# frgfm/Holocron

Measured on AMD Instinct MI355X. Metric: images/sec fwd+bwd+AdaBelief, RepVGG-A0 bs256/GPU 224^2, higher is better.
Workload: dtype bf16; 1 GPU; repvgg_a0 bf16 train step (fwd+bwd+AdaBelief), synthetic 224^2, bs=256 per MI355X (BASELINE.json configs[1]), random-init weights, 10 classes, CE label_smoothing 0.1; global_batch=256, parallelism=dp1, mode=weight gradients on a second stream; hipGraph replay of the full step, dump_outputs=/tmp/code/gt15__hip_graft__frgfm__Holocron/driver_out/dump_parent, deterministic=True

## Files before the change

holocron_amd/_lib.py:

```python
import ctypes as C
import os

import torch

_HERE = os.path.dirname(os.path.abspath(__file__))
LIB_PATH = os.environ.get("HC_LIB_PATH") or os.path.join(_HERE, "lib", "libholocron_hip.so")

HC_MAX_TAPS = 12
HC_MT_CHUNK = 8192
HC_STAT_REPLICAS = 128

c_void_p, c_int32, c_int64, c_float, c_double = C.c_void_p, C.c_int32, C.c_int64, C.c_float, C.c_double


class ConvClass(C.Structure):
    _fields_ = [("OHg", c_int32), ("OWg", c_int32), ("oy0", c_int32), ("ox0", c_int32), ("ostep", c_int32),
                ("istep", c_int32), ("ntaps", c_int32), ("tap", c_int32 * HC_MAX_TAPS)]


class ConvDesc(C.Structure):
    _fields_ = [("src0", c_void_p), ("src1", c_void_p), ("wpk", c_void_p), ("dst", c_void_p), ("resid", c_void_p),
                ("stats", c_void_p), ("bias", c_void_p), ("act", c_int32),
                ("N", c_int32), ("IH", c_int32), ("IW", c_int32), ("srcC", c_int32),
                ("OH", c_int32), ("OW", c_int32), ("Cout", c_int32), ("T", c_int32), ("nclass", c_int32),
# ... 162 lines not shown
    "hc_yolo1_loss_fwd": (c_int32, [c_void_p] * 3 + [c_int32] * 8 + [c_void_p] * 4 + [c_int32] + [c_void_p] * 4),
    "hc_yolo1_loss_bwd": (c_int32, [c_void_p] * 3 + [c_int32] * 8 + [c_void_p] * 4 + [c_int32] + [c_void_p] * 7),
    "hc_yolo1_decode": (c_int32, [c_void_p] * 3 + [c_int32] * 7 + [c_void_p] * 4),
    "hc_yolo_format_fwd": (c_int32, [c_void_p] * 2 + [c_int32] * 7 + [c_void_p] * 5),
    "hc_yolo_format_bwd": (c_int32, [c_void_p] * 3 + [c_int32] * 7 + [c_void_p] * 7),
    "hc_lamb_step": (c_int32, [c_void_p, c_int32, c_void_p, c_void_p, c_void_p, c_int32, c_void_p]),
    "hc_tadam_step": (c_int32, [c_void_p, c_int32, c_void_p, c_void_p, c_void_p, c_void_p, c_void_p, c_void_p, c_int32, c_void_p]),
    "hc_adan_step": (c_int32, [c_void_p, c_void_p, c_int32, c_void_p, c_void_p]),
    "hc_lookahead_sync": (c_int32, [c_void_p, c_int32, c_float, c_void_p]),
    "hc_multi_copy": (c_int32, [C.POINTER(MultiCopyDesc), c_void_p]),
    "hc_msbn_finalize": (c_int32, [C.POINTER(MsbnDesc), c_void_p]),
    "hc_msbn_bwd_finalize": (c_int32, [C.POINTER(MsbnDesc), c_void_p]),
    "hc_msbn_apply": (c_int32, [C.POINTER(MsbnIo), c_void_p, c_void_p, c_void_p, c_int32, c_void_p]),
    "hc_msbn_bwd_reduce": (c_int32, [C.POINTER(MsbnIo), c_void_p, c_int32, c_void_p, c_void_p, c_int32, c_void_p]),
    "hc_msbn_bwd_apply": (c_int32, [C.POINTER(MsbnIo), c_void_p, c_int32, c_void_p, c_void_p, c_int32, c_void_p]),
    "hc_dwrep_dgrad": (c_int32, [c_void_p, c_void_p, c_int32, c_void_p, c_void_p] + [c_int32] * 5 + [c_void_p]),
    "hc_conv_gather": (c_int32, [C.POINTER(ConvDesc), c_void_p]),
    "hc_conv_pointwise_supported": (c_int32, [C.POINTER(ConvDesc)]),
    "hc_conv_pointwise": (c_int32, [C.POINTER(ConvDesc), c_void_p]),
    "hc_conv_small": (c_int32, [C.POINTER(ConvSmallDesc), c_void_p]),
    "hc_conv_small_supported": (c_int32, [C.POINTER(ConvSmallDesc)]),
    "hc_conv_rows_fused_bwd_supported": (c_int32, [C.POINTER(ConvSmallDesc)]),
    "hc_conv_rows_fused_bwd": (c_int32, [C.POINTER(ConvSmallDesc), c_void_p, c_void_p, c_int32] + [c_void_p] * 8),
    "hc_conv_s2_supported": (c_int32, [C.POINTER(ConvS2Desc)]),
    "hc_conv_s2_fwd": (c_int32, [C.POINTER(ConvS2Desc), c_void_p]),
    "hc_conv_s2_dgrad_supported": (c_int32, [C.POINTER(ConvS2DgradDesc)]),
    "hc_conv_s2_dgrad": (c_int32, [C.POINTER(ConvS2DgradDesc), c_void_p]),
    "hc_conv_s2_stem_wgrad_ws_bytes": (c_int64, []),
    "hc_conv_s2_stem_wgrad": (c_int32, [c_void_p] * 6 + [c_int32] * 4 + [c_void_p]),
    "hc_conv_wgrad_ws_bytes": (c_int64, [C.POINTER(WgradDesc)]),
    "hc_conv_wgrad": (c_int32, [C.POINTER(WgradDesc), c_void_p]),
    "hc_conv_wgrad_group_supported": (c_int32, [C.POINTER(WgradGroupDesc)]),
    "hc_conv_wgrad_group_ws_bytes": (c_int64, [C.POINTER(WgradGroupDesc)]),
    "hc_conv_wgrad_group": (c_int32, [C.POINTER(WgradGroupDesc), c_void_p]),
    "hc_rep_wgrad_supported": (c_int32, [C.POINTER(RepWgradDesc)]),
    "hc_rep_wgrad_ws_bytes": (c_int64, [C.POINTER(RepWgradDesc)]),
    "hc_rep_wgrad_plan": (c_int32, [C.POINTER(RepWgradDesc), c_void_p]),
    "hc_rep_wgrad": (c_int32, [C.POINTER(RepWgradDesc), c_void_p]),
    "hc_pack_conv_weight": (c_int32, [c_void_p, c_void_p] + [c_int32] * 7 + [c_void_p]),
    "hc_pack_conv_weights_multi": (c_int32, [c_void_p, c_int32, c_int64, c_void_p]),
    "hc_nchw_to_nhwc_bf16": (c_int32, [c_void_p, c_void_p] + [c_int32] * 5 + [c_void_p]),
    "hc_nhwc_bf16_to_nchw": (c_int32, [c_void_p, c_void_p] + [c_int32] * 5 + [c_void_p]),
    "hc_im2col_small": (c_int32, [c_void_p, c_void_p] + [c_int32] * 11 + [c_void_p]),
    "hc_unpack_im2col_grad": (c_int32, [c_void_p, c_void_p] + [c_int32] * 6 + [c_void_p]),
    "hc_rep_bn_finalize": (c_int32, [C.POINTER(RepBnDesc), c_void_p]),
    "hc_rep_apply": (c_int32, [c_void_p] * 6 + [c_int64, c_int32, c_int32, c_void_p]),
# ... 152 lines not shown
```

holocron_amd/csrc/conv_rows48.hip:

```cpp
#include <type_traits>
#include "common.h"
#include "../../include/holocron_hip.h"

namespace crq {

constexpr int NT = 512, C = 48, CK = 2, PSC = C / 8 + 1, PS = PSC * 16, S3 = 9 * CK, S1 = CK, S = S3 + S1;
static_assert((PS / 8) % 4 == 2, "pixel pitch must be 2 x odd 8-byte units");

struct Args {
    hc_conv_small_desc d;
    int reps;
    int nunits;
    int delay;
};

template <int W>
struct Geo {
    static constexpr int RW = W > 64 ? 1 : 2;
    static constexpr int SEGW = (W + 15) / 16;
    static constexpr int NF = RW * SEGW;
    static constexpr int UR = 4 * RW;
    static constexpr int WW = W + 1;
    static constexpr int NSLOT = (UR + 2) * WW + 1;
    static constexpr int NDMA = (NSLOT * PS + 1023) / 1024;
    static constexpr int WIN = NDMA * 1024;
    static constexpr int SMEM = 2 * WIN + 64 + 1024;
    static_assert(SMEM <= 160 * 1024, "LDS budget");
};

__device__ __forceinline__ u32x4 uniform_rsrc(const void* p, unsigned bytes) {
    const unsigned long long v = reinterpret_cast<unsigned long long>(p);
    u32x4 r;
    r[0] = __builtin_amdgcn_readfirstlane((unsigned)v);
    r[1] = __builtin_amdgcn_readfirstlane((unsigned)(v >> 32) & 0xffffu);
    r[2] = __builtin_amdgcn_readfirstlane(bytes);
    r[3] = 0x00020000u;
    return r;
}
__device__ __forceinline__ bf16x8 frag2(const char* lo_p, const char* hi_p) {
    const u32x2 lo = *reinterpret_cast<const u32x2*>(lo_p), hi = *reinterpret_cast<const u32x2*>(hi_p);
    const u32x4 v = {lo[0], lo[1], hi[0], hi[1]};
    return __builtin_bit_cast(bf16x8, v);
}
__device__ __forceinline__ float row16_sum(float v) {
    v += __builtin_bit_cast(float, __builtin_amdgcn_update_dpp(0, __builtin_bit_cast(int, v), 0x128, 0xf, 0xf, false));
    v += __builtin_bit_cast(float, __builtin_amdgcn_update_dpp(0, __builtin_bit_cast(int, v), 0x124, 0xf, 0xf, false));
    v += __builtin_bit_cast(float, __builtin_amdgcn_update_dpp(0, __builtin_bit_cast(int, v), 0x122, 0xf, 0xf, false));
    v += __builtin_bit_cast(float, __builtin_amdgcn_update_dpp(0, __builtin_bit_cast(int, v), 0x121, 0xf, 0xf, false));
    return v;
}

template <int W, int MODE, int DBG>
__global__ __launch_bounds__(NT, 1) void conv_rows48_kernel(const Args a) {
    using G = Geo<W>;
    constexpr int WW = G::WW, NF = G::NF, UR = G::UR, RW = G::RW, SEGW = G::SEGW;
    extern __shared__ __attribute__((aligned(1024))) char smem[];
    const hc_conv_small_desc& d = a.d;
    const int tid = threadIdx.x, lane = tid & 63;
    const int wid = __builtin_amdgcn_readfirstlane(tid >> 6);
    const int team = wid >> 2, pw = wid & 3;
    const int H = d.H, UPI = H / UR;
    const unsigned lds0 = hc_lds_addr(smem);
    const int px = lane & 15, g = lane >> 4;
    const int region = team * G::WIN;
    int* cnt = reinterpret_cast<int*>(smem + 2 * G::WIN) + team * 8;
    int gen = 0;

    if (tid < 16) reinterpret_cast<int*>(smem + 2 * G::WIN)[tid] = 0;
    __syncthreads();

    auto team_sync = [&]() __attribute__((always_inline)) {
        asm volatile("s_waitcnt vmcnt(0) lgkmcnt(0)" ::: "memory");
        gen += 4;
        if (lane == 0) __hip_atomic_fetch_add(cnt, 1, __ATOMIC_RELAXED, __HIP_MEMORY_SCOPE_WORKGROUP);
        while (__hip_atomic_load(cnt, __ATOMIC_RELAXED, __HIP_MEMORY_SCOPE_WORKGROUP) < gen) __builtin_amdgcn_s_sleep(1);
        asm volatile("" ::: "memory");
    };

    const unsigned act_bytes = (unsigned)d.N * H * W * C * 2u;
    const u32x4 rsA = uniform_rsrc(d.srcA, act_bytes);
    const u32x4 rsB = uniform_rsrc(MODE == 1 ? d.srcB : d.srcA, act_bytes);
    const __amdgpu_buffer_rsrc_t rsw = make_rsrc(d.w3, (unsigned)(S * C * 64));

    const unsigned wl = (unsigned)((lane & 15) * 64 + g * 16);
    u32x4 af[3][3];
    auto load_a = [&](int buf, int s) __attribute__((always_inline)) {
        if (DBG & 4) return;
#pragma unroll
        for (int f = 0; f < 3; ++f) af[buf][f] = buf_load16(rsw, wl, (unsigned)(s * (C * 64) + f * 1024));
    };

    auto stage_window = [&](const u32x4 rs, int n, int row0, int j0, int j1) __attribute__((always_inline)) {
        if (DBG & 8) return;
        const unsigned img = (unsigned)n * (unsigned)(H * W * C * 2);
        for (int j = j0 + pw; j < j1; j += 4) {
            const int J = j * 64 + lane;
            const int slot = J / PSC, c = J - slot * PSC;
            const int r = slot / WW, x = slot - r * WW;
            const int ih = row0 - 1 + r;
            const bool ok = c < PSC - 1 && slot < G::NSLOT && x >= 1 && ih >= 0 && ih < H;
            const unsigned off = img + (unsigned)((ih * W + x - 1) * C * 2 + c * 16);
            hc_dma16(rs, lds0 + (unsigned)(region + j * 1024), ok ? off : HC_OOB);
        }
    };

    const int vb = region + ((pw * RW + 1) * WW + px + 1) * PS + g * 8;
    bf16x8 bfr[2][NF];
    auto load_b = [&](int buf, int bofs, int second) __attribute__((always_inline)) {
        if (DBG & 2) return;
        const char* sb = smem + vb + bofs;
#pragma unroll
        for (int i = 0; i < NF; ++i) {
            const int o = ((i / SEGW) * WW + 16 * (i % SEGW)) * PS;
            bfr[buf][i] = frag2(sb + o, sb + o + second);
        }
    };

    f32x4 acc[3][NF];
    auto zero_acc = [&]() __attribute__((always_inline)) {
#pragma unroll
        for (int f = 0; f < 3; ++f)
#pragma unroll
            for (int i = 0; i < NF; ++i) acc[f][i] = f32x4{0.f, 0.f, 0.f, 0.f};
    };
    auto mfma_step = [&](int ab, int bb) __attribute__((always_inline)) {
#pragma unroll
        for (int i = 0; i < NF; ++i)
#pragma unroll
            for (int f = 0; f < 3; ++f) {
                if (DBG & 1) acc[f][i][0] += __builtin_bit_cast(float, af[ab][f][0]) * (float)bfr[bb][i][0];
                else acc[f][i] = __builtin_amdgcn_mfma_f32_16x16x32_bf16(__builtin_bit_cast(bf16x8, af[ab][f]), bfr[bb][i], acc[f][i], 0, 0, 0);
            }
    };
    auto step = [&](int a3, int par, int s, int bnext, int second_next, bool prefetch) __attribute__((always_inline)) {
        if (s + 2 < S) load_a((a3 + 2) % 3, s + 2);
        if (prefetch) load_b(par ^ 1, bnext, second_next);
        __builtin_amdgcn_sched_barrier(0);
// ... 8 lines not shown
#pragma unroll
            for (int f = 0; f < 3; ++f)
#pragma unroll
                for (int i = 0; i < NF; ++i) t += acc[f][i][0];
            if (t == 123.456f) reinterpret_cast<float*>(outp)[tid] = t;
            return;
        }
        const size_t img = (size_t)n * H * W * C;
        __builtin_amdgcn_sched_barrier(0);
        float st[2][12];
#pragma unroll
        for (int k = 0; k < 2; ++k)
#pragma unroll
            for (int e = 0; e < 12; ++e) st[k][e] = 0.f;
#pragma unroll
        for (int i = 0; i < NF; ++i) {
            const int row = row0 + pw * RW + i / SEGW, col = 16 * (i % SEGW) + px;
            const bool ok = col < W;
            const size_t e0 = img + (size_t)(row * W + (ok ? col : 0)) * C + cbase;
            bf16_t* op = reinterpret_cast<bf16_t*>(outp) + e0;
            const bf16_t* rp = residp != nullptr ? reinterpret_cast<const bf16_t*>(residp) + e0 : nullptr;
            u32x4 r16 = {0u, 0u, 0u, 0u};
            u32x2 r8 = {0u, 0u};
            if (rp != nullptr && ok) {
                r16 = *reinterpret_cast<const u32x4*>(rp);
                r8 = *reinterpret_cast<const u32x2*>(rp + 32 - 4 * g);
            }
            u32x2 pk[3];
#pragma unroll
            for (int f = 0; f < 3; ++f) {
                f32x4 v = acc[f][i];
                if (stats != nullptr) {
#pragma unroll
                    for (int e = 0; e < 4; ++e) {
                        const float x = ok ? v[e] : 0.f;
                        st[0][f * 4 + e] += x;
                        st[1][f * 4 + e] += x * x;
                    }
                }
                const unsigned ra = f == 0 ? r16[0] : (f == 1 ? r16[2] : r8[0]), rb = f == 0 ? r16[1] : (f == 1 ? r16[3] : r8[1]);
                v[0] += bf16lo(ra); v[1] += bf16hi(ra); v[2] += bf16lo(rb); v[3] += bf16hi(rb);
                pk[f] = u32x2{pack_bf16x2(v[0], v[1]), pack_bf16x2(v[2], v[3])};
            }
            if (ok) {
                *reinterpret_cast<u32x4*>(op) = u32x4{pk[0][0], pk[0][1], pk[1][0], pk[1][1]};
                *reinterpret_cast<u32x2*>(op + 32 - 4 * g) = pk[2];
            }
        }
        if (stats != nullptr) {
            float* rep = stats + (size_t)((blockIdx.x * 8 + wid) % a.reps) * 2 * C + cbase;
#pragma unroll
            for (int k = 0; k < 2; ++k) {
                float mine = 0.f;
#pragma unroll
                for (int e = 0; e < 12; ++e) {
                    const float x = row16_sum(st[k][e]);
                    mine = px == e ? x : mine;
                }
                if (px < 12) atomicAdd(rep + k * C + (px < 8 ? px : 24 - 4 * g + px), mine);
            }
        }
    };

    if (team == 1)
        for (int i = 0; i < a.delay; ++i) __builtin_amdgcn_s_sleep(64);
    bool first = true;
    for (int u = 2 * blockIdx.x + team; u < a.nunits; u += 2 * gridDim.x) {
        const int n = u / UPI, row0 = (u - n * UPI) * UR;
        if (!first) team_sync();
        first = false;
        stage_window(rsA, n, row0, 0, G::NDMA);
        load_a(0, 0);
        load_a(1, 1);
        team_sync();
        zero_acc();
        load_b(0, (-WW - 1) * PS, 32);
#pragma nounroll
        for (int kh = 0; kh < 3; ++kh) {
            const int rofs = (kh - 1) * WW * PS;
#pragma unroll
            for (int t = 0; t < 6; ++t) {
                const int kw = t >> 1, kk = t & 1;
                int bnext, second;
                bool pf = true;
                if (kk == 0) { bnext = rofs + (kw - 1) * PS + 64; second = 0; }
                else if (t < 5) { bnext = rofs + kw * PS; second = 32; }
                else {
                    bnext = kh < 2 ? kh * WW * PS - PS : 0;
                    second = 32;
                    pf = kh < 2 || MODE == 0;
                }
                step(t % 3, kk, 6 * kh + t, bnext, second, pf);
            }
        }
        if (MODE == 0) {
            epilogue(d.out3, d.stats3, nullptr, n, row0);
            zero_acc();
        } else {
            team_sync();
            stage_window(rsB, n, row0, (WW * PS) / 1024, ((UR + 1) * WW * PS + PS + 1023) / 1024);
            team_sync();
            load_b(0, 0, 32);
        }
        step(0, 0, S3, 64, 0, true);
        step(1, 1, S3 + 1, 0, 0, false);
        if (MODE == 0) epilogue(d.out1, d.stats1, nullptr, n, row0);
        else epilogue(d.out3, nullptr, d.resid, n, row0);
    }
}

template <int W>
bool shape_ok(const hc_conv_small_desc& d) {
    return d.C == C && d.Cout == C && d.W == W && d.H >= Geo<W>::UR && d.H % Geo<W>::UR == 0 && d.N >= 1 &&
           (double)d.N * d.H * d.W * C * 2.0 < 2147483000.0;
}

template <int W, int MODE, int DBG>
void launch1(const Args& a, hipStream_t st) {
    auto kern = conv_rows48_kernel<W, MODE, DBG>;
    constexpr int smem = Geo<W>::SMEM;
    static bool attr_set = false;
    if (!attr_set) {
        (void)hipFuncSetAttribute(reinterpret_cast<const void*>(kern), hipFuncAttributeMaxDynamicSharedMemorySize, smem);
        attr_set = true;
    }
    int grid = (a.nunits + 1) / 2;
    if (grid > 256) grid = 256;
    hipLaunchKernelGGL(kern, dim3(grid), dim3(NT), smem, st, a);
}

template <int W>
void launch(Args& a, hipStream_t st) {
    static const int dbg = getenv("HC_CRQ_DBG") ? atoi(getenv("HC_CRQ_DBG")) : 0;
    constexpr int delay = 2;
    a.nunits = a.d.N * (a.d.H / Geo<W>::UR);
    a.delay = delay;
    const bool dg = (a.d.mode & 1) == 1;
#define CRQ_CASE(k) case k: if (dg) launch1<W, 1, k>(a, st); else launch1<W, 0, k>(a, st); break;
    switch (dbg) {
        CRQ_CASE(1) CRQ_CASE(2) CRQ_CASE(4) CRQ_CASE(7) CRQ_CASE(8) CRQ_CASE(16) CRQ_CASE(24) CRQ_CASE(31)
        default: if (dg) launch1<W, 1, 0>(a, st); else launch1<W, 0, 0>(a, st); break;
    }
#undef CRQ_CASE
}

}

bool hc_conv_rows48_supported(const hc_conv_small_desc& d) {
    static const int on = [] { const char* e = getenv("HC_CONV_ROWS48"); return e == nullptr ? 1 : atoi(e); }();
    if (on <= 0 || (d.mode & HC_CONV_SMALL_ROWS_IMAGE) == 0 || (d.mode & ~(HC_CONV_SMALL_ROWS_IMAGE | 1)) != 0) return false;
    if ((d.mode & 1) && on < 2) return false;
    return crq::shape_ok<112>(d) || crq::shape_ok<56>(d);
}
int hc_conv_rows48_launch(const hc_conv_small_desc& d, hipStream_t st) {
    if (!hc_conv_rows48_supported(d)) return HC_ERR_ARG;
    const bool dg = (d.mode & 1) == 1;
    if (d.srcA == nullptr || d.w3 == nullptr || d.out3 == nullptr) return HC_ERR_ARG;
    if (!dg && d.out1 == nullptr) return HC_ERR_ARG;
    if (dg && d.srcB == nullptr) return HC_ERR_ARG;
    if (!dg && (d.stats3 == nullptr) != (d.stats1 == nullptr)) return HC_ERR_ARG;
    crq::Args a;
    a.d = d;
    a.reps = hc_get_stat_replicas();
    if (d.W == 112) crq::launch<112>(a, st);
    else crq::launch<56>(a, st);
    return hc_launch_status();
}
```

holocron_amd/nn/repblock_op.py:

```python
import ctypes as C

import os

import torch

from .. import _lib
from .._lib import ConvS2Desc, ConvS2DgradDesc, PackItem, RepBnBwdDesc, RepBnDesc, StemBwdDesc, StemDesc, check, ptr, stream
from ..ops import conv as cv

STEM_KPAD = 32
FUSED_BWD = os.environ.get("HC_REP_FUSED_BWD", "1") != "0"


class ZeroPool:

    def __init__(self):
        self.buf = None
        self.used = 0
        self.high = 0
        self.depth = 0
        self.gen = 0
        self.retired = []
        self.graph_users = 0
        self.buf_captured = False

    def _retire(self):
        if self.buf is not None and self.buf_captured:
            self.retired.append(self.buf)
        self.buf, self.buf_captured = None, False

    def release_retired(self):
        self.graph_users = max(0, self.graph_users - 1)
        if self.graph_users == 0:
            self.retired = []
# ... 85 lines not shown
class RepState:

    def __init__(self, stride, identity):
        self.stride = stride
        self.identity = identity
        self.emit_stats = False
        self.fwd_cache = cv.PackCache()
        self.bwd_cache = cv.PackCache()
        self.desc = {}
        self.bn = None
        self.eps = 1e-5
        self.momentum = 0.1
        self.training = True
        self.last_out_stats = None
        self.packed = None
        self.packed_key = None
        self.pack_table = {}
        self.rows_image = (False, False)
        self.stack_fwd = False
        self.s2 = False
        self.s2_images = None
        self.s2_dgrad = False
        self.s2_dimg = None

    @staticmethod
    def weights_key(w3, w1):
        return (w3.data_ptr(), w3._version, w1.data_ptr(), w1._version, cv.weights_epoch())

    def pack_items(self, w3, w1):
        Cout, Cin = w3.shape[0], w3.shape[1]
        dev = w3.device
        stem = (Cin % 16) != 0
        if self.s2:
            return self._pack_items_s2(w3, w1, Cout, Cin, dev, stem)
        self.stack_fwd = (stem or (self.stride == 2 and Cin <= 48)) and Cout % 4 == 0
        if self.packed is None or self.packed[0].device != dev:
            if self.stack_fwd:
                self.packed = (torch.zeros((2 * Cout, 1, STEM_KPAD) if stem else (2 * Cout, 9, Cin), dtype=torch.bfloat16, device=dev),
                               None, None if stem else torch.empty((Cin, 10, Cout), dtype=torch.bfloat16, device=dev))
            elif any(self.rows_image):
                rf, rb = self.rows_image
                self.packed = (cv.rows_image(Cout, dev) if rf else torch.empty((Cout, 9, Cin), dtype=torch.bfloat16, device=dev),
                               None if rf else torch.empty((Cout, 1, Cin), dtype=torch.bfloat16, device=dev),
                               cv.rows_image(Cout, dev) if rb else torch.empty((Cin, 10, Cout), dtype=torch.bfloat16, device=dev))
            elif stem:
                self.packed = (torch.zeros((Cout, 1, STEM_KPAD), dtype=torch.bfloat16, device=dev),
                               torch.zeros((Cout, 1, STEM_KPAD), dtype=torch.bfloat16, device=dev), None)
            else:
                self.packed = (torch.empty((Cout, 9, Cin), dtype=torch.bfloat16, device=dev),
                               torch.empty((Cout, 1, Cin), dtype=torch.bfloat16, device=dev),
                               torch.empty((Cin, 10, Cout), dtype=torch.bfloat16, device=dev))
            self.packed_key = None
        wp3, wp1, wpd = self.packed
        if self.stack_fwd:
            if stem:
                return [(w3, wp3, Cout, Cin, 3, 3, 2, 0, STEM_KPAD), (w1, wp3[Cout:], Cout, Cin, 1, 1, 2, 4 * Cin, STEM_KPAD)]
            return [(w3, wp3, Cout, Cin, 3, 3, 0, 0, 9), (w1, wp3[Cout:], Cout, Cin, 1, 1, 0, 4, 9),
                    (w3, wpd, Cout, Cin, 3, 3, 1, 0, 10), (w1, wpd, Cout, Cin, 1, 1, 1, 9, 10)]
        if any(self.rows_image):
            rf, rb = self.rows_image
            fwd = ([(w3, wp3, Cout, Cin, 3, 3, 3, 0, 10), (w1, wp3, Cout, Cin, 1, 1, 3, 9, 10)] if rf else
                   [(w3, wp3, Cout, Cin, 3, 3, 0, 0, 9), (w1, wp1, Cout, Cin, 1, 1, 0, 0, 1)])
            bwd = ([(w3, wpd, Cout, Cin, 3, 3, 4, 0, 10), (w1, wpd, Cout, Cin, 1, 1, 4, 9, 10)] if rb else
                   [(w3, wpd, Cout, Cin, 3, 3, 1, 0, 10), (w1, wpd, Cout, Cin, 1, 1, 1, 9, 10)])
            return fwd + bwd
        if stem:
            return [(w3, wp3, Cout, Cin, 3, 3, 2, 0, STEM_KPAD), (w1, wp1, Cout, Cin, 1, 1, 2, 4 * Cin, STEM_KPAD)]
        return [(w3, wp3, Cout, Cin, 3, 3, 0, 0, 9), (w1, wp1, Cout, Cin, 1, 1, 0, 0, 1),
                (w3, wpd, Cout, Cin, 3, 3, 1, 0, 10), (w1, wpd, Cout, Cin, 1, 1, 1, 9, 10)]

    def _pack_items_s2(self, w3, w1, Cout, Cin, dev, stem):
        if stem:
            s3, s1, s1b, mode, tap1 = 2, 1, 0, 6, 4
        else:
            pt = Cin // 8
            s3, s1b, mode, tap1 = (9 * pt + 3) // 4, (9 * pt) // 4, 5, 9 * pt
            s1 = (10 * pt + 3) // 4 - s1b
        if self.s2_images is None or self.s2_images[0].device != dev:
            self.s2_images = (torch.zeros((Cout // 16, s3, 64, 8), dtype=torch.bfloat16, device=dev),
                              torch.zeros((Cout // 16, s1, 64, 8), dtype=torch.bfloat16, device=dev))
            self.packed_key = None
        gather_dgrad = not stem and not self.s2_dgrad
        if self.packed is None or (self.packed[2] is not None) != gather_dgrad or (gather_dgrad and self.packed[2].device != dev):
            self.packed = (None, None, torch.empty((Cin, 10, Cout), dtype=torch.bfloat16, device=dev) if gather_dgrad else None)
            self.packed_key = None
        i3, i1 = self.s2_images
        items = [(w3, i3, Cout, Cin, 3, 3, mode, 0, s3, 0), (w1, i1, Cout, Cin, 1, 1, mode, tap1, s1, s1b)]
        if gather_dgrad:
            wpd = self.packed[2]
            items += [(w3, wpd, Cout, Cin, 3, 3, 1, 0, 10), (w1, wpd, Cout, Cin, 1, 1, 1, 9, 10)]
        elif self.s2_dgrad:
            sd = 10 * (Cout // 8) // 4
# ... 36 lines not shown
                dg = None
            sf = sd = None
            rows = (False, False)
            if Cin % 16 == 0 and s == 1:
                sf = cv.conv_small_desc(N, H, W, Cin, Cout, cv.ROWS_IMAGE)
                sd = cv.conv_small_desc(N, H, W, Cout, Cin, cv.ROWS_IMAGE | 1)
                rows = (sf is not None, sd is not None)
                if sf is None:
                    sf = cv.conv_small_desc(N, H, W, Cin, Cout, 0)
                if sd is None:
                    sd = cv.conv_small_desc(N, H, W, Cout, Cin, 1)
            s2d = None
            if s == 2:
                c = ConvS2Desc()
                c.N, c.H, c.W, c.Cin, c.Cout, c.x_nchw_f32 = N, H, W, Cin, Cout, 1 if Cin % 16 else 0
                if _lib.load().hc_conv_s2_supported(C.byref(c)):
                    s2d = c
            s2g = None
            if s == 2 and s2d is not None and Cin % 16 == 0:
                c = ConvS2DgradDesc()
                c.N, c.H, c.W, c.Cin, c.Cout = N, H, W, Cin, Cout
                if _lib.load().hc_conv_s2_dgrad_supported(C.byref(c)):
                    s2g = c
            self.desc[key] = (f3, f1, dg, sf, sd, rows, s2d, s2g)
        rows = self.desc[key][5]
        s2, s2g = self.desc[key][6] is not None, self.desc[key][7] is not None
        if rows != self.rows_image or s2 != self.s2 or s2g != self.s2_dgrad:
            self.rows_image, self.s2, self.s2_dgrad, self.packed, self.packed_key = rows, s2, s2g, None, None
        return self.desc[key][:5]

    def s2_desc(self, N, Cin, H, W, Cout):
        self.descs(N, Cin, H, W, Cout)
        return self.desc[(N, Cin, H, W, Cout)][6]


def _stats_of(x):
    st = getattr(x, "_hc_stats", None)
    if st is not None:
        return st
    N, Cc, H, W = x.shape
    st = POOL.take((_lib.stat_replicas(), 2, Cc), x.device)
    with cv.profiled("bn_elementwise", 0.0, N * H * W * Cc * 2.0):
        check(_lib.load().hc_channel_stats(ptr(x), ptr(st), N * H * W, Cc, stream()), "hc_channel_stats")
    return st


def block_convs_forward(st, src, w3, w1, geom, stats=None, stem_cin=None):
    N, Cin, H, W, Cout = geom
    f3, f1, _, sf, _ = st.descs(N, Cin, H, W, Cout)
    OH, OW = f3.OH, f3.OW
    dev = src.device
# ... 12 lines not shown
        nbytes = src.numel() * src.element_size() + 2 * y3.numel() * 2.0
        with cv.profiled("conv_s2", flops, nbytes):
            check(_lib.load().hc_conv_s2_fwd(C.byref(s2d), stream()), "hc_conv_s2_fwd")
        return y3, y1
    fl3 = fl1 = None
    if stem_cin is not None:
        fl3, fl1 = 2.0 * N * OH * OW * Cout * 9 * stem_cin, 2.0 * N * OH * OW * Cout * stem_cin
    s3 = None if stats is None else stats[0]
    s1 = None if stats is None else stats[1]
    if sf is not None:
        cv.launch_conv_small_fwd(sf, src, wp3, wp1, y3, y1, s3, s1)
    elif st.stack_fwd:
        f31 = st.stacked_desc(N, Cin, H, W, Cout)
        cv.launch_conv(f31, src, wp3, y3, stats=s3, dst2=y1, stats2=s1, co_split=Cout,
                       flops=None if fl3 is None else fl3 + fl1)
    else:
        cv.launch_conv(f3, src, wp3, y3, stats=s3, flops=fl3)
        cv.launch_conv(f1, src, wp1, y1, stats=s1, flops=fl1)
    return y3, y1


def block_dgrad(st, dy3, dy1, dxid, w3, w1, geom):
    N, Cin, H, W, Cout = geom
    _, _, dg, _, sdg = st.descs(N, Cin, H, W, Cout)
    wpd = st.ensure_packed(w3, w1)[2]
    dx = cv.empty_cl(N, Cin, H, W, dy3.device)
    s2g = st.desc[(N, Cin, H, W, Cout)][7]
    if s2g is not None:
        if dxid is not None:
            raise _lib.HipError("stride-2 data gradient: a stride-2 RepBlock has no identity branch")
        s2g.dy3, s2g.dy1, s2g.wimg, s2g.dx = ptr(dy3), ptr(dy1), ptr(st.s2_dimg), ptr(dx)
        with cv.profiled("conv_s2", 2.0 * N * dy3.shape[2] * dy3.shape[3] * Cout * 10 * Cin, dx.numel() * 2.0 + 2 * dy3.numel() * 2.0):
            check(_lib.load().hc_conv_s2_dgrad(C.byref(s2g), stream()), "hc_conv_s2_dgrad")
        return dx
    if sdg is not None:
        cv.launch_conv_small_dgrad(sdg, dy3, dy1, wpd, dx, resid=dxid)
    else:
        cv.launch_conv(dg, dy3, wpd, dx, src1=dy1, resid=dxid)
    return dx


def fused_dgrad_desc(st, geom):
    N, Cin, H, W, Cout = geom
    sdg = st.descs(N, Cin, H, W, Cout)[4]
    if sdg is None or not st.rows_image[1] or Cin != Cout or not _lib.load().hc_conv_rows_fused_bwd_supported(C.byref(sdg)):
        return None
    return sdg


def block_dgrad_fused(st, sdg, g, coef, act, y3, y1, x, bcoef, w3, w1, bufs=None):
    wpd = st.ensure_packed(w3, w1)[2]
    dy3, dy1, dxid, dx = bufs if bufs is not None else (torch.empty_like(y3), torch.empty_like(y1), torch.empty_like(x), torch.empty_like(x))
    sdg.srcA, sdg.srcB, sdg.resid, sdg.w3, sdg.w1, sdg.out3, sdg.out1, sdg.stats3, sdg.stats1 = None, None, None, ptr(wpd), None, ptr(dx), None, None, None
    tb = x.numel() * 2.0
    with cv.profiled("conv_rows", 2.0 * sdg.N * sdg.H * sdg.W * sdg.Cout * 10 * sdg.C, 8 * tb):
        check(_lib.load().hc_conv_rows_fused_bwd(C.byref(sdg), ptr(g), ptr(coef), act, ptr(y3), ptr(y1), ptr(x), ptr(bcoef), ptr(dy3),
                                                 ptr(dy1), ptr(dxid), stream()), "hc_conv_rows_fused_bwd")
    return dy3, dy1, dxid, dx


def block_wgrad(st, src, dy3, dy1, w3, w1, geom, stem_cin=None, defer=False):
    N, Cin, H, W, Cout = geom
    lib = _lib.load()
    npix = dy3.shape[0] * dy3.shape[2] * dy3.shape[3]
    if stem_cin is not None and src.dtype == torch.float32:
        dw3 = torch.empty_like(w3, dtype=torch.float32)
        dw1 = torch.empty_like(w1, dtype=torch.float32)
        ws = torch.empty((int(lib.hc_conv_s2_stem_wgrad_ws_bytes()),), dtype=torch.uint8, device=src.device)
        with cv.profiled("conv_wgrad", 2.0 * npix * Cout * 10 * stem_cin, src.numel() * 4.0 + 2 * dy3.numel() * 2.0):
            rc = lib.hc_conv_s2_stem_wgrad(ptr(src), ptr(dy3), ptr(dy1), ptr(dw3), ptr(dw1), ptr(ws), N, H, W, 0, stream())
        if rc == 0:
            return dw3, dw1
        src = cv.im2col_small(src, 3, 3, st.stride, 1, STEM_KPAD)
    if stem_cin is not None:
        K = STEM_KPAD
        dwc3 = cv.conv_wgrad(src, dy3, K, Cout, 1, 1, 1, 0, flops=2.0 * npix * Cout * 9 * stem_cin)
        dwc1 = cv.conv_wgrad(src, dy1, K, Cout, 1, 1, 1, 0, flops=2.0 * npix * Cout * stem_cin)
        dw3 = torch.empty_like(w3, dtype=torch.float32)
        check(lib.hc_unpack_im2col_grad(ptr(dwc3), ptr(dw3), Cout, stem_cin, 3, 3, K, 0, stream()), "hc_unpack_im2col_grad")
        dw1 = dwc1.view(Cout, K)[:, 4 * stem_cin:5 * stem_cin].reshape(Cout, stem_cin, 1, 1).contiguous()
# ... 199 lines not shown
```

include/holocron_hip.h:

```cpp
#ifndef HOLOCRON_HIP_H
#define HOLOCRON_HIP_H
#include <stdint.h>
#ifdef __cplusplus
extern "C" {
#endif

typedef void* hc_stream_t;

#define HC_MAX_TAPS 12
#define HC_STAT_REPLICAS 128
#define HC_STAT_REPLICAS_DETERMINISTIC 32768
int hc_set_deterministic(int on);
int hc_get_deterministic(void);
int hc_get_stat_replicas(void);

typedef struct {
    int32_t OHg, OWg, oy0, ox0, ostep, istep, ntaps;
    int32_t tap[HC_MAX_TAPS];
} hc_conv_class;
#define HC_TAP(dy, dx, src, wt) \
    ((int32_t)(((uint32_t)(dy) & 0xffu) | (((uint32_t)(dx) & 0xffu) << 8) | ((uint32_t)(src) << 16) | ((uint32_t)(wt) << 24)))

typedef struct {
    const void* src0;
// ... 23 lines not shown
int hc_conv_gather(const hc_conv_desc* d, hc_stream_t stream);
int hc_conv_pointwise_supported(const hc_conv_desc* d);
int hc_conv_pointwise(const hc_conv_desc* d, hc_stream_t stream);

#define HC_CONV_SMALL_ROWS_IMAGE 4
typedef struct {
    const void* srcA;
    const void* srcB;
    const void* w3;
    const void* w1;
    void* out3;
    void* out1;
    const void* resid;
    float* stats3;
    float* stats1;
    int32_t w3_rstride, w1_rstride;
    int32_t N, H, W, C, Cout, mode;
} hc_conv_small_desc;
int hc_conv_small(const hc_conv_small_desc* d, hc_stream_t stream);
int hc_conv_small_supported(const hc_conv_small_desc* d);
int hc_conv_rows_fused_bwd_supported(const hc_conv_small_desc* d);
int hc_conv_rows_fused_bwd(const hc_conv_small_desc* d, const void* g, const float* coef, int32_t act, const void* y3, const void* y1,
                           const void* x, const float* bcoef, void* dy3, void* dy1, void* dxid, hc_stream_t stream);

typedef struct {
    const void* x;
    const void* w3img;
    const void* w1img;
    void* y3;
    void* y1;
    float* stats3;
    float* stats1;
    int32_t N, H, W, Cin, Cout, x_nchw_f32;
} hc_conv_s2_desc;
int hc_conv_s2_supported(const hc_conv_s2_desc* d);
int hc_conv_s2_fwd(const hc_conv_s2_desc* d, hc_stream_t stream);
typedef struct {
    const void* dy3;
    const void* dy1;
    const void* wimg;
    void* dx;
    int32_t N, H, W, Cin, Cout;
} hc_conv_s2_dgrad_desc;
int hc_conv_s2_dgrad_supported(const hc_conv_s2_dgrad_desc* d);
int hc_conv_s2_dgrad(const hc_conv_s2_dgrad_desc* d, hc_stream_t stream);
int64_t hc_conv_s2_stem_wgrad_ws_bytes(void);
// ... 452 lines not shown
```

Baseline: 26110 images/sec.

## Fuse RepVGG backward elementwise into 48-channel rows dgrad kernel

Adds a MODE 2 variant of the 48-channel rows conv kernel. Its prologue computes the block's backward elementwise step (activation gradient and per-branch dy3/dy1/dxid) straight from g, y3, y1 and x into the LDS window and stores those branches to global memory, then runs the 3x3+1x1 dgrad on them. This removes a separate elementwise pass and a restaging read. Each team now handles a contiguous run of row units so it can carry halo rows between units instead of re-staging them. The Python side turns it on by default for identity 48-channel blocks at width 112 and later, at the cost of more kernel complexity, register pressure, and load imbalance from the contiguous split.

Result: no change. 26360 images/sec (median of 6 runs) (+1.0%).

```diff
diff --git a/holocron_amd/_lib.py b/holocron_amd/_lib.py
--- a/holocron_amd/_lib.py
+++ b/holocron_amd/_lib.py
@@ -208,6 +208,10 @@
     "hc_conv_small_supported": (c_int32, [C.POINTER(ConvSmallDesc)]),
     "hc_conv_rows_fused_bwd_supported": (c_int32, [C.POINTER(ConvSmallDesc)]),
     "hc_conv_rows_fused_bwd": (c_int32, [C.POINTER(ConvSmallDesc), c_void_p, c_void_p, c_int32] + [c_void_p] * 8),
+    "hc_conv_rows48_fused_bwd_supported": (c_int32, [C.POINTER(ConvSmallDesc)]),
+    "hc_conv_rows48_fused_bwd": (c_int32, [C.POINTER(ConvSmallDesc), c_void_p, c_void_p, c_int32] + [c_void_p] * 8),
+    "hc_conv_rows48_fused_bwd_plan": (c_int32, [C.POINTER(ConvSmallDesc), c_int32, c_void_p]),
+    "hc_conv_rows48_dgrad": (c_int32, [C.POINTER(ConvSmallDesc), c_void_p]),
     "hc_conv_s2_supported": (c_int32, [C.POINTER(ConvS2Desc)]),
     "hc_conv_s2_fwd": (c_int32, [C.POINTER(ConvS2Desc), c_void_p]),
     "hc_conv_s2_dgrad_supported": (c_int32, [C.POINTER(ConvS2DgradDesc)]),
diff --git a/holocron_amd/csrc/conv_rows48.hip b/holocron_amd/csrc/conv_rows48.hip
--- a/holocron_amd/csrc/conv_rows48.hip
+++ b/holocron_amd/csrc/conv_rows48.hip
@@ -1,5 +1,6 @@
 #include <type_traits>
 #include "common.h"
+#include "rep_ew.h"
 #include "../../include/holocron_hip.h"
 
 namespace crq {
@@ -13,6 +14,25 @@
     int nunits;
     int delay;
 };
+
+struct FusedArgs : Args {
+    const void *g, *y3, *y1, *x;
+    const float *coef, *bcoef;
+    void* dy3;
+    int act;
+};
+
+__host__ __device__ inline void team_run(int nunits, int teams, int t, int& start, int& count) {
+    const int base = nunits / teams, rem = nunits % teams;
+    start = t * base + (t < rem ? t : rem);
+    count = base + (t < rem ? 1 : 0);
+}
+inline int fused_grid(int nunits, int grid_cap) {
+    int grid = (nunits + 1) / 2;
+    if (grid > 256) grid = 256;
+    if (grid_cap > 0 && grid > grid_cap) grid = grid_cap;
+    return grid;
+}
 
 template <int W>
 struct Geo {
@@ -42,6 +62,9 @@
     const u32x4 v = {lo[0], lo[1], hi[0], hi[1]};
     return __builtin_bit_cast(bf16x8, v);
 }
+__device__ __forceinline__ u32x2 ld8_l2(__amdgpu_buffer_rsrc_t r, unsigned voff, unsigned soff) {
+    return __builtin_bit_cast(u32x2, __builtin_amdgcn_raw_buffer_load_b64(r, voff, soff, 16));
+}
 __device__ __forceinline__ float row16_sum(float v) {
     v += __builtin_bit_cast(float, __builtin_amdgcn_update_dpp(0, __builtin_bit_cast(int, v), 0x128, 0xf, 0xf, false));
     v += __builtin_bit_cast(float, __builtin_amdgcn_update_dpp(0, __builtin_bit_cast(int, v), 0x124, 0xf, 0xf, false));
@@ -51,7 +74,7 @@
 }
 
 template <int W, int MODE, int DBG>
-__global__ __launch_bounds__(NT, 1) void conv_rows48_kernel(const Args a) {
+__global__ __launch_bounds__(NT, 1) void conv_rows48_kernel(const std::conditional_t<MODE == 2, FusedArgs, Args> a) {
     using G = Geo<W>;
     constexpr int WW = G::WW, NF = G::NF, UR = G::UR, RW = G::RW, SEGW = G::SEGW;
     extern __shared__ __attribute__((aligned(1024))) char smem[];
@@ -79,7 +102,7 @@
 
     const unsigned act_bytes = (unsigned)d.N * H * W * C * 2u;
     const u32x4 rsA = uniform_rsrc(d.srcA, act_bytes);
-    const u32x4 rsB = uniform_rsrc(MODE == 1 ? d.srcB : d.srcA, act_bytes);
+    const u32x4 rsB = uniform_rsrc(MODE != 0 ? d.srcB : d.srcA, act_bytes);
     const __amdgpu_buffer_rsrc_t rsw = make_rsrc(d.w3, (unsigned)(S * C * 64));
 
     const unsigned wl = (unsigned)((lane & 15) * 64 + g * 16);
@@ -104,6 +127,104 @@
         }
     };
 
+    auto fused_prologue = [&](int n, int row0, bool carry, bool next_carry) __attribute__((always_inline)) {
+        if constexpr (MODE == 2) {
+            if (DBG & 32) return;
+            constexpr int CG = C / 8, PPS = 256 / CG, BATCH = 2;
+            const int rb = carry ? 2 : 0;
+            int lane = tid & 63;
+            asm volatile("" : "+v"(lane));
+            if (!carry || row0 + UR >= H) {
+                const int slot_lo = carry ? (UR + 1) * WW : 0;
+                for (int j = (slot_lo * PS) / 1024 + pw; j < G::NDMA; j += 4) {
+                    const int J = j * 64 + lane;
+                    const int slot = J / PSC, c = J - slot * PSC;
+                    const int r = slot / WW, x = slot - r * WW;
+                    const int ih = row0 - 1 + r;
+                    const bool ok = c < PSC - 1 && slot < G::NSLOT && x >= 1 && ih >= 0 && ih < H;
+                    if (!ok && slot >= slot_lo) *reinterpret_cast<u32x4*>(smem + region + J * 16) = u32x4{0u, 0u, 0u, 0u};
+                }
+            }
+            const int tt = pw * 64 + lane;
+            const int pl = tt / CG, chunk = tt - pl * CG;
+            const bool active = pl < PPS;
+            int c0 = chunk * 8;
+            asm volatile("" : "+v"(c0));
+            float a3[8], a1[8], a0[8], sh[8], A3[8], B3[8], C3[8], A1[8], B1[8], C1[8], A0[8], B0[8], C0[8];
+            load8f(a.coef + c0, a3); load8f(a.coef + C + c0, a1); load8f(a.coef + 2 * C + c0, a0); load8f(a.coef + 3 * C + c0, sh);
+            load8f(a.bcoef + 0 * C + c0, A3); load8f(a.bcoef + 1 * C + c0, B3); load8f(a.bcoef + 2 * C + c0, C3);
+            load8f(a.bcoef + 3 * C + c0, A1); load8f(a.bcoef + 4 * C + c0, B1); load8f(a.bcoef + 5 * C + c0, C1);
+            load8f(a.bcoef + 6 * C + c0, A0); load8f(a.bcoef + 7 * C + c0, B0); load8f(a.bcoef + 8 * C + c0, C0);
+            const __amdgpu_buffer_rsrc_t rg = make_rsrc(a.g, act_bytes), r3 = make_rsrc(a.y3, act_bytes), r1 = make_rsrc(a.y1, act_bytes),
+                                         rx = make_rsrc(a.x, act_bytes), rd3 = make_rsrc(a.dy3, act_bytes),
+                                         rd1 = make_rsrc(d.srcB, act_bytes), rd0 = make_rsrc(d.resid, act_bytes);
+            const int HW = H * W, NP = (UR + 2 - rb) * W;
+            const int gp0 = (row0 - 1 + rb) * W;
+            const int st_lo = rb == 0 ? W : 0, st_hi = (UR + 1 + (next_carry ? 1 : 0) - rb) * W;
+            const int act = a.act;
+            struct Batch { u32x4 vg[BATCH], v3[BATCH], v1[BATCH], vx[BATCH]; unsigned off[BATCH]; };
+            auto request = [&](Batch& q, int pb) __attribute__((always_inline)) {
+#pragma unroll
+                for (int b = 0; b < BATCH; ++b) {
+                    const int p = pb + b * PPS, gp = gp0 + p;
+                    const bool ok = active && p < NP && gp >= 0 && gp < HW;
+                    q.off[b] = ok ? (unsigned)(((n * HW + gp) * CG + chunk) * 16) : HC_OOB;
+                    q.vg[b] = buf_load16(rg, q.off[b]);
+                    q.v3[b] = buf_load16(r3, q.off[b]);
+                    q.v1[b] = buf_load16(r1, q.off[b]);
+                    q.vx[b] = buf_load16(rx, q.off[b]);
+                }
+            };
+            auto finish = [&](const Batch& q, int pb) __attribute__((always_inline)) {
+#pragma unroll
+                for (int b = 0; b < BATCH; ++b) {
+                    const int p = pb + b * PPS;
+                    float fg[8], f3[8], f1[8], f0[8], o3[8], o1[8], o0[8];
+                    unpack8(q.vg[b], fg); unpack8(q.v3[b], f3); unpack8(q.v1[b], f1); unpack8(q.vx[b], f0);
+#pragma unroll
+                    for (int i = 0; i < 8; ++i) {
+                        const float fo = act == 1 ? rep_preact<true>(a3[i], f3[i], a1[i], f1[i], a0[i], f0[i], sh[i]) : 1.f;
+                        const float dz = rep_bwd_dz(fo, fg[i]);
+                        o3[i] = rep_bwd_branch(A3[i], dz, B3[i], f3[i], C3[i]);
+                        o1[i] = rep_bwd_branch(A1[i], dz, B1[i], f1[i], C1[i]);
+                        o0[i] = rep_bwd_branch(A0[i], dz, B0[i], f0[i], C0[i]);
+                    }
+                    const u32x4 p3 = pack8(o3);
+                    if (q.off[b] != HC_OOB) {
+                        const int r = p / W, x = p - r * W;
+                        *reinterpret_cast<u32x4*>(smem + region + ((rb + r) * WW + x + 1) * PS + chunk * 16) = p3;
+                    }
+                    const unsigned so = (p >= st_lo && p < st_hi) ? q.off[b] : HC_OOB;
+                    __builtin_amdgcn_raw_buffer_store_b128(p3, rd3, so, 0, 0);
+                    __builtin_amdgcn_raw_buffer_store_b128(pack8(o1), rd1, so, 0, 0);
+                    __builtin_amdgcn_raw_buffer_store_b128(pack8(o0), rd0, so, 0, 0);
+                }
+            };
+            constexpr int STEP = BATCH * PPS;
+            Batch q0, q1;
+            request(q0, pl);
+#pragma nounroll
+            for (int pb = pl; pb < NP + pl; pb += 2 * STEP) {
+                request(q1, pb + STEP);
+                __builtin_amdgcn_sched_barrier(0);
+                finish(q0, pb);
+                __builtin_amdgcn_sched_barrier(0);
+                request(q0, pb + 2 * STEP);
+                __builtin_amdgcn_sched_barrier(0);
+                finish(q1, pb + STEP);
+                __builtin_amdgcn_sched_barrier(0);
+            }
+        }
+    };
+    auto carry_rows = [&]() __attribute__((always_inline)) {
+        if constexpr (MODE == 2) {
+            if (DBG & 32) return;
+            char* wb = smem + region;
+            for (int i = pw * 64 + lane; i < 2 * WW * PS / 16; i += 256)
+                *reinterpret_cast<u32x4*>(wb + i * 16) = *reinterpret_cast<const u32x4*>(wb + UR * WW * PS + i * 16);
+        }
+    };
+
     const int vb = region + ((pw * RW + 1) * WW + px + 1) * PS + g * 8;
     bf16x8 bfr[2][NF];
     auto load_b = [&](int buf, int bofs, int second) __attribute__((always_inline)) {
@@ -113,6 +234,22 @@
         for (int i = 0; i < NF; ++i) {
             const int o = ((i / SEGW) * WW + 16 * (i % SEGW)) * PS;
             bfr[buf][i] = frag2(sb + o, sb + o + second);
+        }
+    };
+
+    auto load_b1 = [&](int n, int row0) __attribute__((always_inline)) {
+        if constexpr (MODE == 2) {
+            if (DBG & 2) return;
+            const __amdgpu_buffer_rsrc_t rd1 = make_rsrc(d.srcB, act_bytes);
+            const unsigned vo = (unsigned)(((n * H + row0 + pw * RW) * W + px) * (C * 2) + g * 8);
+            const unsigned vo_last = (SEGW - 1) * 16 + px < W ? vo : HC_OOB;
+#pragma unroll
+            for (int i = 0; i < NF; ++i) {
+                const unsigned v = (i % SEGW == SEGW - 1) ? vo_last : vo, so = (unsigned)(((i / SEGW) * W + 16 * (i % SEGW)) * (C * 2));
+                const u32x2 lo = ld8_l2(rd1, v, so), hi = ld8_l2(rd1, v, so + 32), k1 = ld8_l2(rd1, v, so + 64);
+                bfr[0][i] = __builtin_bit_cast(bf16x8, u32x4{lo[0], lo[1], hi[0], hi[1]});
+                bfr[1][i] = __builtin_bit_cast(bf16x8, u32x4{k1[0], k1[1], k1[0], k1[1]});
+            }
         }
     };
 
@@ -167,7 +304,13 @@
             const bf16_t* rp = residp != nullptr ? reinterpret_cast<const bf16_t*>(residp) + e0 : nullptr;
             u32x4 r16 = {0u, 0u, 0u, 0u};
             u32x2 r8 = {0u, 0u};
-            if (rp != nullptr && ok) {
+            if (MODE == 2 && rp != nullptr) {
+                const __amdgpu_buffer_rsrc_t rd0 = make_rsrc(residp, act_bytes);
+                const unsigned v = ok ? (unsigned)(e0 * 2) : HC_OOB;
+                const u32x2 ra = ld8_l2(rd0, v, 0), rb = ld8_l2(rd0, v, 8);
+                r16 = u32x4{ra[0], ra[1], rb[0], rb[1]};
+                r8 = ld8_l2(rd0, ok ? (unsigned)(e0 * 2) + 64u - 8u * g : HC_OOB, 0);
+            } else if (rp != nullptr && ok) {
                 r16 = *reinterpret_cast<const u32x4*>(rp);
                 r8 = *reinterpret_cast<const u32x2*>(rp + 32 - 4 * g);
             }
@@ -210,11 +353,16 @@
     if (team == 1)
         for (int i = 0; i < a.delay; ++i) __builtin_amdgcn_s_sleep(64);
     bool first = true;
-    for (int u = 2 * blockIdx.x + team; u < a.nunits; u += 2 * gridDim.x) {
+    int run0 = 0, run_n = 0;
+    if (MODE == 2) team_run(a.nunits, 2 * gridDim.x, 2 * blockIdx.x + team, run0, run_n);
+    const int u_end = MODE == 2 ? run0 + run_n : a.nunits;
+    for (int u = MODE == 2 ? run0 : 2 * blockIdx.x + team; u < u_end; u += MODE == 2 ? 1 : 2 * gridDim.x) {
         const int n = u / UPI, row0 = (u - n * UPI) * UR;
+        const bool carry = MODE == 2 && !first && row0 != 0, next_carry = MODE == 2 && u + 1 < u_end && row0 + UR < H;
         if (!first) team_sync();
         first = false;
-        stage_window(rsA, n, row0, 0, G::NDMA);
+        if (MODE == 2) fused_prologue(n, row0, carry, next_carry);
+        else stage_window(rsA, n, row0, 0, G::NDMA);
         load_a(0, 0);
         load_a(1, 1);
         team_sync();
@@ -241,13 +389,17 @@
         if (MODE == 0) {
             epilogue(d.out3, d.stats3, nullptr, n, row0);
             zero_acc();
-        } else {
+        } else if (MODE == 1) {
             team_sync();
             stage_window(rsB, n, row0, (WW * PS) / 1024, ((UR + 1) * WW * PS + PS + 1023) / 1024);
             team_sync();
             load_b(0, 0, 32);
-        }
-        step(0, 0, S3, 64, 0, true);
+        } else {
+            load_b1(n, row0);
+            team_sync();
+            if (next_carry) carry_rows();
+        }
+        step(0, 0, S3, 64, 0, MODE != 2);
         step(1, 1, S3 + 1, 0, 0, false);
         if (MODE == 0) epilogue(d.out1, d.stats1, nullptr, n, row0);
         else epilogue(d.out3, nullptr, d.resid, n, row0);
@@ -272,6 +424,31 @@
     int grid = (a.nunits + 1) / 2;
     if (grid > 256) grid = 256;
     hipLaunchKernelGGL(kern, dim3(grid), dim3(NT), smem, st, a);
+}
+
+template <int W, int DBG>
+void launch_fused1(const FusedArgs& a, int grid, hipStream_t st) {
+    auto kern = conv_rows48_kernel<W, 2, DBG>;
+    constexpr int smem = Geo<W>::SMEM;
+    static bool attr_set = false;
+    if (!attr_set) {
+        (void)hipFuncSetAttribute(reinterpret_cast<const void*>(kern), hipFuncAttributeMaxDynamicSharedMemorySize, smem);
+        attr_set = true;
+    }
+    hipLaunchKernelGGL(kern, dim3(grid), dim3(NT), smem, st, a);
+}
+template <int W>
+void launch_fused(FusedArgs& a, int grid_cap, hipStream_t st) {
+    static const int dbg = getenv("HC_CRQ_DBG") ? atoi(getenv("HC_CRQ_DBG")) : 0;
+    a.nunits = a.d.N * (a.d.H / Geo<W>::UR);
+    a.delay = 2;
+    const int grid = fused_grid(a.nunits, grid_cap);
+#define CRQ_CASE(k) case k: launch_fused1<W, k>(a, grid, st); break;
+    switch (dbg) {
+        CRQ_CASE(1) CRQ_CASE(2) CRQ_CASE(4) CRQ_CASE(7) CRQ_CASE(8) CRQ_CASE(16) CRQ_CASE(24) CRQ_CASE(31) CRQ_CASE(32)
+        default: launch_fused1<W, 0>(a, grid, st); break;
+    }
+#undef CRQ_CASE
 }
 
 template <int W>
@@ -297,8 +474,20 @@
     if ((d.mode & 1) && on < 2) return false;
     return crq::shape_ok<112>(d) || crq::shape_ok<56>(d);
 }
+static bool rows48_shape_and_mode(const hc_conv_small_desc& d) {
+    if ((d.mode & HC_CONV_SMALL_ROWS_IMAGE) == 0 || (d.mode & ~(HC_CONV_SMALL_ROWS_IMAGE | 1)) != 0) return false;
+    return crq::shape_ok<112>(d) || crq::shape_ok<56>(d);
+}
+static int rows48_launch_checked(const hc_conv_small_desc& d, hipStream_t st);
 int hc_conv_rows48_launch(const hc_conv_small_desc& d, hipStream_t st) {
     if (!hc_conv_rows48_supported(d)) return HC_ERR_ARG;
+    return rows48_launch_checked(d, st);
+}
+extern "C" int hc_conv_rows48_dgrad(const hc_conv_small_desc* dp, hc_stream_t stream) {
+    if (dp == nullptr || dp->mode != (HC_CONV_SMALL_ROWS_IMAGE | 1) || !rows48_shape_and_mode(*dp)) return HC_ERR_ARG;
+    return rows48_launch_checked(*dp, (hipStream_t)stream);
+}
+static int rows48_launch_checked(const hc_conv_small_desc& d, hipStream_t st) {
     const bool dg = (d.mode & 1) == 1;
     if (d.srcA == nullptr || d.w3 == nullptr || d.out3 == nullptr) return HC_ERR_ARG;
     if (!dg && d.out1 == nullptr) return HC_ERR_ARG;
@@ -311,3 +500,41 @@
     else crq::launch<56>(a, st);
     return hc_launch_status();
 }
+
+extern "C" int hc_conv_rows48_fused_bwd_supported(const hc_conv_small_desc* dp) {
+    return dp != nullptr && dp->mode == (HC_CONV_SMALL_ROWS_IMAGE | 1) && rows48_shape_and_mode(*dp) ? 1 : 0;
+}
+extern "C" int hc_conv_rows48_fused_bwd_plan(const hc_conv_small_desc* dp, int32_t grid_cap, int32_t* out) {
+    if (!hc_conv_rows48_fused_bwd_supported(dp) || out == nullptr) return HC_ERR_ARG;
+    const int ur = dp->W == 112 ? crq::Geo<112>::UR : crq::Geo<56>::UR;
+    const int upi = dp->H / ur, nunits = dp->N * upi;
+    const int grid = crq::fused_grid(nunits, grid_cap), teams = 2 * grid;
+    out[0] = grid; out[1] = teams; out[2] = nunits; out[3] = upi;
+    for (int t = 0; t < teams; ++t) {
+        int start, count;
+        crq::team_run(nunits, teams, t, start, count);
+        out[4 + 2 * t] = start;
+        out[5 + 2 * t] = count;
+    }
+    return HC_OK;
+}
+extern "C" int hc_conv_rows48_fused_bwd(const hc_conv_small_desc* dp, const void* g, const float* coef, int32_t act, const void* y3,
+                                        const void* y1, const void* x, const float* bcoef, void* dy3, void* dy1, void* dxid,
+                                        hc_stream_t stream) {
+    if (!hc_conv_rows48_fused_bwd_supported(dp)) return HC_ERR_ARG;
+    if (dp->w3 == nullptr || dp->out3 == nullptr || g == nullptr || coef == nullptr || y3 == nullptr || y1 == nullptr || x == nullptr ||
+        bcoef == nullptr || dy3 == nullptr || dy1 == nullptr || dxid == nullptr || (act != 0 && act != 1))
+        return HC_ERR_ARG;
+    const char* e_grid = getenv("HC_CONV_ROWS48_GRID");
+    const int grid_cap = e_grid ? atoi(e_grid) : 0;
+    crq::FusedArgs a;
+    a.d = *dp;
+    a.d.srcA = dy3;
+    a.d.srcB = dy1;
+    a.d.resid = dxid;
+    a.reps = hc_get_stat_replicas();
+    a.g = g; a.y3 = y3; a.y1 = y1; a.x = x; a.coef = coef; a.bcoef = bcoef; a.dy3 = dy3; a.act = act;
+    if (dp->W == 112) crq::launch_fused<112>(a, grid_cap, (hipStream_t)stream);
+    else crq::launch_fused<56>(a, grid_cap, (hipStream_t)stream);
+    return hc_launch_status();
+}
diff --git a/holocron_amd/nn/repblock_op.py b/holocron_amd/nn/repblock_op.py
--- a/holocron_amd/nn/repblock_op.py
+++ b/holocron_amd/nn/repblock_op.py
@@ -10,6 +10,8 @@
 
 STEM_KPAD = 32
 FUSED_BWD = os.environ.get("HC_REP_FUSED_BWD", "1") != "0"
+FUSED_BWD48 = int(os.environ.get("HC_REP_FUSED_BWD48", "1") or 0)
+FUSED_BWD48_MIN_W = 112
 
 
 class ZeroPool:
@@ -141,6 +143,8 @@
         self.s2_images = None
         self.s2_dgrad = False
         self.s2_dimg = None
+        self.fused48 = False
+        self.fused_img = None
 
     @staticmethod
     def weights_key(w3, w1):
@@ -182,11 +186,22 @@
                    [(w3, wp3, Cout, Cin, 3, 3, 0, 0, 9), (w1, wp1, Cout, Cin, 1, 1, 0, 0, 1)])
             bwd = ([(w3, wpd, Cout, Cin, 3, 3, 4, 0, 10), (w1, wpd, Cout, Cin, 1, 1, 4, 9, 10)] if rb else
                    [(w3, wpd, Cout, Cin, 3, 3, 1, 0, 10), (w1, wpd, Cout, Cin, 1, 1, 1, 9, 10)])
-            return fwd + bwd
+            return fwd + bwd + self._fused48_items(w3, w1, Cout, Cin, dev)
         if stem:
             return [(w3, wp3, Cout, Cin, 3, 3, 2, 0, STEM_KPAD), (w1, wp1, Cout, Cin, 1, 1, 2, 4 * Cin, STEM_KPAD)]
         return [(w3, wp3, Cout, Cin, 3, 3, 0, 0, 9), (w1, wp1, Cout, Cin, 1, 1, 0, 0, 1),
-                (w3, wpd, Cout, Cin, 3, 3, 1, 0, 10), (w1, wpd, Cout, Cin, 1, 1, 1, 9, 10)]
+                (w3, wpd, Cout, Cin, 3, 3, 1, 0, 10), (w1, wpd, Cout, Cin, 1, 1, 1, 9, 10)] + self._fused48_items(w3, w1, Cout, Cin, dev)
+
+    def _fused48_items(self, w3, w1, Cout, Cin, dev):
+        if not self.fused48 or self.rows_image[1]:
+            return []
+        if self.fused_img is None or self.fused_img.device != dev:
+            self.fused_img = cv.rows_image(Cout, dev)
+            self.packed_key = None
+        return [(w3, self.fused_img, Cout, Cin, 3, 3, 4, 0, 10), (w1, self.fused_img, Cout, Cin, 1, 1, 4, 9, 10)]
+
+    def fused_dgrad_image(self):
+        return self.packed[2] if self.rows_image[1] else self.fused_img
 
     def _pack_items_s2(self, w3, w1, Cout, Cin, dev, stem):
         if stem:
@@ -269,11 +284,20 @@
                 c.N, c.H, c.W, c.Cin, c.Cout = N, H, W, Cin, Cout
                 if _lib.load().hc_conv_s2_dgrad_supported(C.byref(c)):
                     s2g = c
-            self.desc[key] = (f3, f1, dg, sf, sd, rows, s2d, s2g)
+            f48 = None
+            if self.identity and s == 1 and Cin == Cout == 48:
+                c = _lib.ConvSmallDesc()
+                c.N, c.H, c.W, c.C, c.Cout, c.mode = N, H, W, Cout, Cin, cv.ROWS_IMAGE | 1
+                if _lib.load().hc_conv_rows48_fused_bwd_supported(C.byref(c)):
+                    f48 = c
+            self.desc[key] = (f3, f1, dg, sf, sd, rows, s2d, s2g, f48)
         rows = self.desc[key][5]
         s2, s2g = self.desc[key][6] is not None, self.desc[key][7] is not None
-        if rows != self.rows_image or s2 != self.s2 or s2g != self.s2_dgrad:
-            self.rows_image, self.s2, self.s2_dgrad, self.packed, self.packed_key = rows, s2, s2g, None, None
+        f48 = self.desc[key][8] is not None and FUSED_BWD and (int(FUSED_BWD48) >= 2 or (int(FUSED_BWD48) == 1 and W >= FUSED_BWD48_MIN_W))
+        if rows != self.rows_image or s2 != self.s2 or s2g != self.s2_dgrad or f48 != self.fused48:
+            self.rows_image, self.s2, self.s2_dgrad, self.fused48, self.packed, self.packed_key = rows, s2, s2g, f48, None, None
+        if f48:
+            return self.desc[key][:4] + (self.desc[key][8],)
         return self.desc[key][:5]
 
     def s2_desc(self, N, Cin, H, W, Cout):
@@ -332,7 +356,8 @@
 
 def block_dgrad(st, dy3, dy1, dxid, w3, w1, geom):
     N, Cin, H, W, Cout = geom
-    _, _, dg, _, sdg = st.descs(N, Cin, H, W, Cout)
+    dg = st.descs(N, Cin, H, W, Cout)[2]
+    sdg = st.desc[(N, Cin, H, W, Cout)][4]
     wpd = st.ensure_packed(w3, w1)[2]
     dx = cv.empty_cl(N, Cin, H, W, dy3.device)
     s2g = st.desc[(N, Cin, H, W, Cout)][7]
@@ -353,19 +378,24 @@
 def fused_dgrad_desc(st, geom):
     N, Cin, H, W, Cout = geom
     sdg = st.descs(N, Cin, H, W, Cout)[4]
+    if st.fused48:
+        return sdg
     if sdg is None or not st.rows_image[1] or Cin != Cout or not _lib.load().hc_conv_rows_fused_bwd_supported(C.byref(sdg)):
         return None
     return sdg
 
 
 def block_dgrad_fused(st, sdg, g, coef, act, y3, y1, x, bcoef, w3, w1, bufs=None):
-    wpd = st.ensure_packed(w3, w1)[2]
+    st.ensure_packed(w3, w1)
+    wpd = st.fused_dgrad_image()
+    lib = _lib.load()
+    entry, name = ((lib.hc_conv_rows48_fused_bwd, "hc_conv_rows48_fused_bwd") if sdg.C == 48 else
+                   (lib.hc_conv_rows_fused_bwd, "hc_conv_rows_fused_bwd"))
     dy3, dy1, dxid, dx = bufs if bufs is not None else (torch.empty_like(y3), torch.empty_like(y1), torch.empty_like(x), torch.empty_like(x))
     sdg.srcA, sdg.srcB, sdg.resid, sdg.w3, sdg.w1, sdg.out3, sdg.out1, sdg.stats3, sdg.stats1 = None, None, None, ptr(wpd), None, ptr(dx), None, None, None
     tb = x.numel() * 2.0
     with cv.profiled("conv_rows", 2.0 * sdg.N * sdg.H * sdg.W * sdg.Cout * 10 * sdg.C, 8 * tb):
-        check(_lib.load().hc_conv_rows_fused_bwd(C.byref(sdg), ptr(g), ptr(coef), act, ptr(y3), ptr(y1), ptr(x), ptr(bcoef), ptr(dy3),
-                                                 ptr(dy1), ptr(dxid), stream()), "hc_conv_rows_fused_bwd")
+        check(entry(C.byref(sdg), ptr(g), ptr(coef), act, ptr(y3), ptr(y1), ptr(x), ptr(bcoef), ptr(dy3), ptr(dy1), ptr(dxid), stream()), name)
     return dy3, dy1, dxid, dx
 
 
diff --git a/include/holocron_hip.h b/include/holocron_hip.h
--- a/include/holocron_hip.h
+++ b/include/holocron_hip.h
@@ -69,6 +69,11 @@
 int hc_conv_rows_fused_bwd_supported(const hc_conv_small_desc* d);
 int hc_conv_rows_fused_bwd(const hc_conv_small_desc* d, const void* g, const float* coef, int32_t act, const void* y3, const void* y1,
                            const void* x, const float* bcoef, void* dy3, void* dy1, void* dxid, hc_stream_t stream);
+int hc_conv_rows48_fused_bwd_supported(const hc_conv_small_desc* d);
+int hc_conv_rows48_fused_bwd(const hc_conv_small_desc* d, const void* g, const float* coef, int32_t act, const void* y3, const void* y1,
+                             const void* x, const float* bcoef, void* dy3, void* dy1, void* dxid, hc_stream_t stream);
+int hc_conv_rows48_fused_bwd_plan(const hc_conv_small_desc* d, int32_t grid_cap, int32_t* out);
+int hc_conv_rows48_dgrad(const hc_conv_small_desc* d, hc_stream_t stream);
 
 typedef struct {
     const void* x;
```
